# xrgtn/x264-i386pic

Measured on AMD Instinct MI355X. Metric: SAD+SATD candidate-MVs/sec + DCT+quant blocks/sec, 1080p, 1/2/4/8 GPU, higher is better.
Workload: dtype u8; 1 GPU; configs[1]: 1920x1080 luma, full-search ME range 16, sad_16x16 candidate tables, 128 frame pairs per GPU per step; mbs_per_frame=8160, candidates_per_mb=1089, parallelism=frame-per-GPU x1, world_size=1

## Files before the change

x264-i386pic_amd/csrc/me.hip:

```cpp
#include "hipcommon.h"
#include <mutex>
#include <string.h>
#include <stdlib.h>
#include <atomic>
#include <utility>

namespace x264hip {

template <int BD, int R, int P, int Y>
__device__ __forceinline__ void me_row( const typename PT<BD>::pixel *rb, intptr_t rs,
                                        const uint32_t (&F)[16][16 / PT<BD>::PPD], uint32_t (&acc)[16],
                                        typename PT<BD>::sadt *out )
{
    constexpr int NDW = 16 / PT<BD>::PPD;
    constexpr int C0 = Y - 15 > 0 ? Y - 15 : 0;
    constexpr int C1 = Y < 2 * R ? Y : 2 * R;
    uint32_t rr[NDW];
    load_packed<NDW>( rb + (intptr_t)Y * rs, rr );
#pragma unroll
    for( int c = C0; c <= C1; c++ )
    {
        const int r = Y - c;
        uint32_t a = r == 0 ? 0u : acc[c & 15];
#pragma unroll
// ... 479 lines not shown
__global__ __launch_bounds__( 256 ) void me_full_sad16_v5_kernel( const uint16_t *__restrict__ fenc, intptr_t fs,
                                                                  intptr_t ffs, const uint16_t *__restrict__ ref,
                                                                  intptr_t rs, intptr_t rfs, int mbw, int mbh,
                                                                  int nframes, uint32_t *__restrict__ table,
                                                                  const int16_t *__restrict__ centre,
                                                                  int16_t *__restrict__ origin, int xcd )
{
    const me_lane l = me_lane_of<2 * G, true>( xcd, nframes, mbh, mbw );
    if( !l.live )
        return;

    uint32_t F[8][8];
    load_fenc( F, (const uint32_t *)(fenc + l.f * ffs + (intptr_t)(16 * l.mby + 8 * l.h) * fs + 16 * l.mbx),
               (int)(fs / 2) );
    int ox, oy;
    me_window<10, R, P>( centre, l.mb, l.mbx, l.mby, mbw, mbh, ox, oy );
    if( origin && l.grp == 0 && l.h == 0 )
    {
        origin[2 * l.mb] = (int16_t)ox;
        origin[2 * l.mb + 1] = (int16_t)oy;
    }
    const uint32_t *rbase = (const uint32_t *)(ref + l.f * rfs + (intptr_t)(16 * l.mby + 8 * l.h + oy) * rs +
                                               16 * l.mbx + ox + 2 * l.grp);
    uint32_t *out = table + l.mb * ((2 * R + 1) * P) + 2 * l.grp;
    if constexpr( P > 2 * G )
    {
        const int c = 2 * l.grp + l.h;
        if( c <= 2 * R )
            *(uint2 *)(table + l.mb * ((2 * R + 1) * P) + c * P + 2 * G) = make_uint2( 0u, 0u );
    }
    auto store = [out]( int c, uint32_t a0, uint32_t a1 ) { *(uint2 *)(out + c * P) = make_uint2( a0, a1 ); };
    ring_p<ME_LEAD> ring;
    fold_pair fold( F, store );
    me_walk<R, 8, ME_LEAD>( rbase, (int)(rs / 2), ring, fold );
}

template <int R>
__global__ __launch_bounds__( 256 ) void me_full_sad8q_v5_kernel( const uint16_t *__restrict__ fenc, intptr_t fs,
                                                                  intptr_t ffs, const uint16_t *__restrict__ ref,
                                                                  intptr_t rs, intptr_t rfs, int mbw, int mbh,
                                                                  int nframes, uint16_t *__restrict__ table8, int xcd )
{
    constexpr int G = R + 1, P = full_pitch( R );
    const me_lane l = me_lane_of<2 * G, true>( xcd, nframes, mbh, mbw );
    if( !l.live )
        return;
    uint32_t F[8][8];
    load_fenc( F, (const uint32_t *)(fenc + l.f * ffs + (intptr_t)(16 * l.mby + 8 * l.h) * fs + 16 * l.mbx),
               (int)(fs / 2) );
    const uint32_t *rbase = (const uint32_t *)(ref + l.f * rfs + (intptr_t)(16 * l.mby + 8 * l.h - R) * rs +
                                               16 * l.mbx - R + 2 * l.grp);
    uint32_t *ql = (uint32_t *)(table8 + (l.mb * 4 + 2 * l.h) * ((2 * R + 1) * P) + 2 * l.grp);
    uint32_t *qr = ql + (2 * R + 1) * P / 2;
    static_assert( P == 2 * G + 2, "one padding dword per row" );
    for( int c = l.grp; c <= 2 * R; c += G )
    {
        ql[c * (P / 2) + G - l.grp] = 0u;
        qr[c * (P / 2) + G - l.grp] = 0u;
    }
    auto store = [ql, qr]( int c, uint32_t left, uint32_t right ) {
        ql[c * (P / 2)] = left;
        qr[c * (P / 2)] = right;
    };
    ring_p<ME_LEAD> ring;
    fold_quad fold( F, store );
    me_walk<R, 8, ME_LEAD>( rbase, (int)(rs / 2), ring, fold );
}

template <int BD>
hipError_t launch_me_full8( const typename PT<BD>::pixel *fenc, intptr_t fs, intptr_t ffs,
                            const typename PT<BD>::pixel *ref, intptr_t rs, intptr_t rfs, int mbw, int mbh,
                            int nframes, int range, uint16_t *table8, hipStream_t stream )
{
    constexpr int PSZ = sizeof( typename PT<BD>::pixel );
    const int64_t lanes = (int64_t)nframes * mbh * mbw * (BD == 8 ? full_pitch( range ) / 4 : 2 * (range + 1));
    if( lanes <= 0 )
        return hipSuccess;
    if( lanes >= (1ll << 32) || (((uintptr_t)fenc | (uintptr_t)ref | (uintptr_t)(fs * PSZ) | (uintptr_t)(rs * PSZ) |
                                  (uintptr_t)table8) & 3) )
        return hipErrorInvalidValue;
    dim3 blk( 256 ), g( (unsigned)((lanes + 255) / 256) );
    const int xcd = me_xcd();
    switch( range )
    {
#define ME8_CASE( R )                                                                                           \
        case R:                                                                                                 \
            if constexpr( BD == 8 )                                                                             \
                hipLaunchKernelGGL( ( me_full_sad8q_kernel<R> ), g, blk, 0, stream, fenc, fs, ffs, ref, rs, rfs, \
                                    mbw, mbh, nframes, table8, xcd );                                           \
            else                                                                                                \
                hipLaunchKernelGGL( ( me_full_sad8q_v5_kernel<R> ), g, blk, 0, stream, fenc, fs, ffs, ref, rs,  \
                                    rfs, mbw, mbh, nframes, table8, xcd );                                      \
            break;
        ME8_CASE( 4 ) ME8_CASE( 8 ) ME8_CASE( 16 ) ME8_CASE( 24 )
#undef ME8_CASE
        default: return hipErrorInvalidValue;
    }
    return hipGetLastError();
}
X264HIP_INSTANTIATE( launch_me_full8 );

template <int BD>
hipError_t launch_me_full( const typename PT<BD>::pixel *fenc, intptr_t fs, intptr_t ffs,
                           const typename PT<BD>::pixel *ref, intptr_t rs, intptr_t rfs, int mbw, int mbh,
                           int nframes, int range, typename PT<BD>::sadt *table, const int16_t *centre,
                           int16_t *origin, hipStream_t stream )
{
    constexpr int PSZ = sizeof( typename PT<BD>::pixel );
    const bool cen = centre != nullptr;
    const int64_t nmb = (int64_t)nframes * mbh * mbw;
    if( nmb <= 0 )
        return hipSuccess;
    const int ncol = cen ? cen_pitch( BD, range ) : 2 * range + 1;
    const int64_t groups = BD == 8 ? al4( ncol ) / 4 : 2 * (cen ? cen_cols( 10, range ) / 2 : range + 1);
    bool grouped = !(((uintptr_t)fenc | (uintptr_t)ref | (uintptr_t)(fs * PSZ) | (uintptr_t)(rs * PSZ)) & 3);
    if( nmb * groups >= (1ll << 32) )
        grouped = false;
    const bool share = grouped && BD == 8 && !cen && (range == 8 || range == 16);
    const int64_t lanes = nmb * (share ? groups - 1 : grouped ? groups : ncol);
    dim3 blk( 256 ), g( (unsigned)((lanes + 255) / 256) );
    const int xcd = me_xcd();
    switch( range )
    {
#define ME_GO( R, CEN )                                                                                           \
    if( !grouped )                                                                                                \
        hipLaunchKernelGGL( ( me_full_sad16_kernel<BD, R, CEN ? cen_pitch( BD, R ) : 2 * R + 1> ), g, blk, 0,    \
                            stream, fenc, fs, ffs, ref, rs, rfs, mbw, mbh, nframes, table, centre, origin );      \
    else if constexpr( BD == 8 && !CEN && cs_range<R>() )                                                         \
        hipLaunchKernelGGL( ( me_full_sad16_v7_kernel<R, full_pitch( R ) / 4, cs_lanes<R>()> ), g, blk, 0,        \
                            stream, fenc, fs, ffs, ref, rs, rfs, mbw, mbh, nframes, table, centre, origin, xcd ); \
    else if constexpr( BD == 8 )                                                                                  \
        hipLaunchKernelGGL( ( me_full_sad16_v7_kernel<R, (CEN ? cen_pitch( 8, R ) : full_pitch( R )) / 4> ), g,   \
                            blk, 0, stream, fenc, fs, ffs, ref, rs, rfs, mbw, mbh, nframes, table, centre, origin, \
                            xcd );                                                                                \
    else                                                                                                          \
        hipLaunchKernelGGL( ( me_full_sad16_v5_kernel<R, CEN ? cen_cols( 10, R ) / 2 : R + 1,                     \
                                                      CEN ? cen_pitch( 10, R ) : full_pitch( R )> ),              \
                            g, blk, 0, stream, fenc, fs, ffs, ref, rs, rfs, mbw, mbh, nframes, table, centre,     \
                            origin, xcd );
#define ME_CASE( R )                                                                                              \
        case R:                                                                                                   \
            if( cen ) { ME_GO( R, true ) } else { ME_GO( R, false ) }                                             \
            break;
        ME_CASE( 4 ) ME_CASE( 8 ) ME_CASE( 16 ) ME_CASE( 24 )
#undef ME_CASE
#undef ME_GO
        default: return hipErrorInvalidValue;
    }
    return hipGetLastError();
}

X264HIP_INSTANTIATE( launch_me_full );

template <int R> constexpr int esa7_groups() { return ((((2 * R + 3) & ~3) + 3) + 3) / 4; }
template <int R> constexpr int esa7_mbs() { return 256 / esa7_groups<R>(); }
constexpr int esa7_groups_rt( int R ) { return ((((2 * R + 3) & ~3) + 3) + 3) / 4; }
template <int R, bool TAB>
__global__ __launch_bounds__( 256 ) void me_full_esa_v7_kernel( const uint8_t *__restrict__ fenc, intptr_t fs,
                                                                intptr_t ffs, const uint8_t *__restrict__ ref,
                                                                intptr_t rs, intptr_t rfs, int mbw, int mbh,
                                                                int nframes, int me_range,
                                                                const int16_t *__restrict__ par,
                                                                const uint16_t *__restrict__ cost_mv,
                                                                uint32_t *__restrict__ keys, int xcd,
                                                                uint16_t *__restrict__ tab,
                                                                int16_t *__restrict__ torg,
                                                                const int32_t *__restrict__ init_cost )
{
    constexpr int G = esa7_groups<R>();
    constexpr int P = cen_pitch( 8, R );
    constexpr int W = 2 * R + 1;
    constexpr int MPW = esa7_mbs<R>();
    constexpr int NSP = 256 - MPW * G;
    constexpr int SP = W | 1;
    __shared__ uint32_t s_row[MPW * SP];
    __shared__ uint32_t s_need[MPW];
    __shared__ uint32_t s_key[MPW];
    const uint32_t nmb = (uint32_t)nframes * (uint32_t)mbh * (uint32_t)mbw;
    const int tid = (int)threadIdx.x;
    const bool spare = tid >= MPW * G;
    const uint32_t wg0 = (xcd ? xcd_block( blockIdx.x, gridDim.x ) : blockIdx.x) * MPW;

    int lmb, grp, mbx, mby, bmx, bmy, min_x, min_y, max_x, max_y, width, ox, oy;
    int64_t mb, f;
    bool live;
    const uint16_t *cx, *cy;
    auto setup = [&]( int slot ) __attribute__( ( always_inline ) ) {
        lmb = slot;
        const uint32_t mbr = wg0 + (uint32_t)slot;
        live = mbr < nmb;
        const uint32_t mb32 = min( mbr, nmb - 1 ), t32 = mb32 / (uint32_t)mbw, f32 = t32 / (uint32_t)mbh;
        mbx = (int)(mb32 - t32 * (uint32_t)mbw);
        mby = (int)(t32 - f32 * (uint32_t)mbh);
        mb = mb32;
        f = f32;
        const int16_t *p = par + 8 * mb;
        bmx = p[0];
        bmy = p[1];
        min_x = max( bmx - me_range, (int)p[4] );
        min_y = max( bmy - me_range, (int)p[5] );
        max_x = min( bmx + me_range, (int)p[6] );
        max_y = min( bmy + me_range, (int)p[7] );
        width = (max_x - min_x + 3) & ~3;
        cx = cost_mv - p[2];
        cy = cost_mv - p[3];
        const int16_t cen[2] = { (int16_t)bmx, (int16_t)bmy };
        me_window<8, R, P>( cen, 0, mbx, mby, mbw, mbh, ox, oy );
    };
    setup( spare ? 0 : tid / G );
    grp = spare ? G : tid - lmb * G;
    const bool need = live && min_x + width - 1 - ox >= 4 * G;
    if( !spare && grp == 0 )
    {
        s_need[lmb] = need;
        s_key[lmb] = 0xFFFFFFFFu;
    }
    if( TAB && !spare && live && grp == 0 )
    {
        torg[2 * mb] = (int16_t)ox;
        torg[2 * mb + 1] = (int16_t)oy;
    }
    if( !TAB && !spare && live )
    {
        uint32_t *srow = s_row + lmb * SP;
#pragma unroll
        for( int c0 = 0; c0 < W; c0 += G )
        {
            const int c = c0 + grp, my = oy + c;
            if( c < W )
                srow[c] = my >= min_y && my <= max_y
                              ? ((uint32_t)cy[4 * my] << 12) + (uint32_t)((my - min_y) * width)
                              : 0xFFFFFFFFu;
        }
    }
    __syncthreads();
    bool twice = false;
    if constexpr( NSP > 0 )
    {
        if( spare )
        {
            int k = tid - MPW * G, slot = -1;
            for( int i = 0; i < MPW && slot < 0; i++ )
                if( s_need[i] && k-- == 0 )
                    slot = i;
            if( slot >= 0 )
                setup( slot );
            else
                live = false;
        }
        else if( grp == 0 && need )
        {
            int rank = 0;
            for( int i = 0; i < lmb; i++ )
                rank += s_need[i] ? 1 : 0;
            twice = rank >= NSP;
        }
    }
    else
        twice = !spare && grp == 0 && need;

    uint32_t F[16][4];
    load_fenc( F, (const uint32_t *)(fenc + f * ffs + (intptr_t)(16 * mby) * fs + 16 * mbx), (int)(fs / 4) );
    const uint32_t *rmb = (const uint32_t *)(ref + f * rfs + (intptr_t)(16 * mby + oy) * rs + 16 * mbx + ox);
    uint32_t ck[4];
    auto columns = [&]( int g ) __attribute__( ( always_inline ) ) {
#pragma unroll
        for( int k = 0; k < 4; k++ )
        {
            const int mx = ox + 4 * g + k;
            const bool in = mx >= min_x && mx < min_x + width;
            ck[k] = in ? ((uint32_t)cx[mx * 4] << 12) + (uint32_t)(mx - min_x) : 0xF0000000u;
        }
    };
    columns( grp );
    uint32_t key = 0xFFFFFFFFu;
    uint32_t *srow = s_row + lmb * SP;
    auto reduce = [&]( int c, uint32_t lo, uint32_t hi ) {
        __attribute__( ( address_space( 3 ) ) ) uint32_t *q = (__attribute__( ( address_space( 3 ) ) ) uint32_t *)srow;
        asm volatile( "" : "+v"( q ) );
        const uint32_t S = q[c];
        uint32_t w0 = lo & 0xffff, w1 = lo >> 16, w2 = hi & 0xffff, w3 = hi >> 16;
        asm( "" : "+v"( w0 ), "+v"( w1 ), "+v"( w2 ), "+v"( w3 ) );
        const uint32_t k0 = __builtin_elementwise_add_sat( (w0 << 12) + ck[0], S );
        const uint32_t k1 = __builtin_elementwise_add_sat( (w1 << 12) + ck[1], S );
        const uint32_t k2 = __builtin_elementwise_add_sat( (w2 << 12) + ck[2], S );
        const uint32_t k3 = __builtin_elementwise_add_sat( (w3 << 12) + ck[3], S );
        key = min( min( key, k0 ), k1 );
        key = min( min( key, k2 ), k3 );
        asm volatile( "" : "+v"( key ) );
    };
    ring_q<ME_LEAD> ring;
    if constexpr( TAB )
    {
        uint64_t *out = (uint64_t *)(tab + mb * ((2 * R + 1) * P) + 4 * grp);
        auto store = [&out]( int c, uint32_t lo, uint32_t hi ) { out[c * (P / 4)] = ((uint64_t)hi << 32) | lo; };
        fold_row fold( F, store );
        if( live )
        {
            me_walk<R, 16, ME_LEAD>( rmb + grp, (int)(rs / 4), ring, fold );
            if( twice )
            {
                out = (uint64_t *)(tab + mb * ((2 * R + 1) * P) + 4 * G);
                me_walk<R, 16, ME_LEAD>( rmb + G, (int)(rs / 4), ring, fold );
            }
        }
    }
    else
    {
        fold_row fold( F, reduce );
        me_walk<R, 16, ME_LEAD>( rmb + grp, (int)(rs / 4), ring, fold );
        if( twice )
        {
            columns( G );
            me_walk<R, 16, ME_LEAD>( rmb + G, (int)(rs / 4), ring, fold );
        }
        if( live && key < 0xF0000000u )
            atomicMin( &s_key[lmb], key );
        __syncthreads();
        if( tid < MPW && wg0 + (uint32_t)tid < nmb )
        {
            const int64_t i = wg0 + (uint32_t)tid;
            const int16_t *q = par + 8 * i;
            const int qx = q[0], qy = q[1];
            const int mnx = max( qx - me_range, (int)q[4] ), mny = max( qy - me_range, (int)q[5] );
            const int wd = (min( qx + me_range, (int)q[6] ) - mnx + 3) & ~3;
            const uint32_t k = s_key[tid];
            int32_t bc = init_cost[i], rx = qx, ry = qy;
            if( k != 0xFFFFFFFFu && (int32_t)(k >> 12) < bc )
            {
                const int ki = (int)(k & 4095);
                bc = (int32_t)(k >> 12);
                ry = mny + ki / wd;
                rx = mnx + ki % wd;
            }
            keys[3 * i] = (uint32_t)bc;
            keys[3 * i + 1] = (uint32_t)rx;
            keys[3 * i + 2] = (uint32_t)ry;
        }
    }
}

__global__ __launch_bounds__( 256 ) void me_esa_finish_kernel( int nmb, int me_range, const int16_t *__restrict__ par,
                                                               const int32_t *__restrict__ init_cost,
                                                               int32_t *__restrict__ out )
{
    const int i = blockIdx.x * blockDim.x + threadIdx.x;
    if( i >= nmb )
        return;
    const int16_t *p = par + 8 * i;
    const int bmx = p[0], bmy = p[1];
    const int min_x = max( bmx - me_range, (int)p[4] ), min_y = max( bmy - me_range, (int)p[5] );
    const int max_x = min( bmx + me_range, (int)p[6] );
    const int width = (max_x - min_x + 3) & ~3;
    const uint32_t key = (uint32_t)out[3 * i];
    int32_t bcost = init_cost[i], rx = bmx, ry = bmy;
    if( key != 0xFFFFFFFFu && (int32_t)(key >> 12) < bcost )
    {
        const int k = (int)(key & 4095);
        bcost = (int32_t)(key >> 12);
        ry = min_y + k / width;
        rx = min_x + k % width;
    }
    out[3 * i] = bcost;
    out[3 * i + 1] = rx;
    out[3 * i + 2] = ry;
}

template <int R>
__global__ __launch_bounds__( 256 ) void me_full_esa_v5_kernel( const uint16_t *__restrict__ fenc, intptr_t fs,
                                                                intptr_t ffs, const uint16_t *__restrict__ ref,
                                                                intptr_t rs, intptr_t rfs, int mbw, int mbh,
                                                                int nframes, int me_range,
                                                                const int16_t *__restrict__ par,
                                                                const uint16_t *__restrict__ cost_mv,
                                                                uint32_t *__restrict__ keys, int xcd )
{
    constexpr int G = cen_cols( 10, R ) / 2;
    constexpr int P = cen_pitch( 10, R );
    const int64_t slot = (int64_t)(xcd ? xcd_block( blockIdx.x, gridDim.x ) : blockIdx.x) * blockDim.x + threadIdx.x;
    const int64_t total = (int64_t)nframes * mbh * mbw * (2 * G);
    if( slot >= total )
        return;
    const int h = (int)(slot & 1);
    const int grp = (int)((slot >> 1) % G);
    const int64_t mb = slot / (2 * G);
    const int mbx = (int)(mb % mbw);
    const int64_t t = mb / mbw;
    const int mby = (int)(t % mbh);
    const int64_t f = t / mbh;

    uint32_t F[8][8];
    load_fenc( F, (const uint32_t *)(fenc + f * ffs + (intptr_t)(16 * mby + 8 * h) * fs + 16 * mbx), (int)(fs / 2) );
    const int16_t *p = par + 8 * mb;
    const int bmx = p[0], bmy = p[1];
    const int min_x = max( bmx - me_range, (int)p[4] ), min_y = max( bmy - me_range, (int)p[5] );
    const int max_x = min( bmx + me_range, (int)p[6] ), max_y = min( bmy + me_range, (int)p[7] );
    const int width = (max_x - min_x + 3) & ~3;
    const uint16_t *cx = cost_mv - p[2], *cy = cost_mv - p[3];
    int ox, oy;
    const int16_t cen[2] = { (int16_t)bmx, (int16_t)bmy };
    me_window<10, R, P>( cen, 0, mbx, mby, mbw, mbh, ox, oy );
    const uint32_t *rbase =
        (const uint32_t *)(ref + f * rfs + (intptr_t)(16 * mby + 8 * h + oy) * rs + 16 * mbx + ox + 2 * grp);
    const int mxc = ox + 2 * grp + h;
    const bool cin = mxc >= min_x && mxc < min_x + width;
    const uint32_t cinv = cin ? 0u : 0xFFFFFFFFu;
    const int ccost = cin ? (int)cx[mxc * 4] : 0;
    uint32_t key = 0xFFFFFFFFu;
    const int ibase = mxc - min_x - min_y * width;
    uint32_t ynext = cy[4 * min( max( oy, min_y ), max_y )];
    auto reduce = [&]( int c, uint32_t a0, uint32_t a1 ) {
        const int my = oy + c;
        const uint32_t rinv = my >= min_y && my <= max_y ? 0u : 0xFFFFFFFFu;
        const uint32_t ycost = ynext;
        int yi = 4 * min( max( my + 1, min_y ), max_y );
        asm volatile( "" : "+v"( yi ) );
        ynext = cy[yi];
        const uint32_t sad = h ? a1 : a0;
        const uint32_t k = ((sad + (uint32_t)ccost + ycost) << 12) | (uint32_t)(my * width + ibase);
        key = min( key, k | cinv | rinv );
        asm volatile( "" : "+v"( key ) );
    };
    ring_p<ME_LEAD> ring;
    fold_pair fold( F, reduce );
    me_walk<R, 8, ME_LEAD>( rbase, (int)(rs / 2), ring, fold );
    key = min( key, (uint32_t)__builtin_amdgcn_update_dpp( (int)0xFFFFFFFF, (int)key, 0xB1, 0xF, 0xF, false ) );
    if( !h && key != 0xFFFFFFFFu )
        atomicMin( keys + 3 * mb, key );
}

template <int BD>
hipError_t launch_me_search_esa( const typename PT<BD>::pixel *fenc, intptr_t fs, intptr_t ffs,
                                 const typename PT<BD>::pixel *ref, intptr_t rs, intptr_t rfs, int mbw, int mbh,
                                 int nframes, int range, int me_range, const int16_t *par, const int32_t *init_cost,
                                 const uint16_t *cost_mv, int32_t *out, hipStream_t stream )
{
    const int64_t nmb = (int64_t)nframes * mbw * mbh;
    if( nmb <= 0 )
        return hipSuccess;
    if( nmb > 0x7fffffff ||
        (((uintptr_t)fenc | (uintptr_t)ref | (uintptr_t)(fs * sizeof( typename PT<BD>::pixel )) |
          (uintptr_t)(rs * sizeof( typename PT<BD>::pixel ))) & 3) )
        return hipErrorInvalidValue;
    if( BD != 8 )
    {
        const hipError_t e = hipMemsetAsync( out, 0xFF, (size_t)nmb * 3 * sizeof( int32_t ), stream );
        if( e != hipSuccess )
            return e;
    }
    const int64_t mpw = range == 4 ? esa7_mbs<4>() : range == 8 ? esa7_mbs<8>() : range == 16 ? esa7_mbs<16>()
                                                                                               : esa7_mbs<24>();
    const int64_t lanes = nmb * 2 * (cen_cols( 10, range ) / 2);
    dim3 blk( 256 ), g( (unsigned)(BD == 8 ? (nmb + mpw - 1) / mpw : (lanes + 255) / 256) );
    const int xcd = me_xcd();
    switch( range )
    {
#define ESA_CASE( R )                                                                                             \
        case R:                                                                                                   \
            if constexpr( BD == 8 )                                                                               \
                hipLaunchKernelGGL( ( me_full_esa_v7_kernel<R, false> ), g, blk, 0, stream, fenc, fs, ffs, ref, rs, \
                                    rfs, mbw, mbh, nframes, me_range, par, cost_mv, (uint32_t *)out, xcd,         \
                                    nullptr, nullptr, init_cost );                                                \
            else                                                                                                  \
                hipLaunchKernelGGL( ( me_full_esa_v5_kernel<R> ), g, blk, 0, stream, fenc, fs, ffs, ref, rs, rfs, \
                                    mbw, mbh, nframes, me_range, par, cost_mv, (uint32_t *)out, xcd );            \
            break;
        ESA_CASE( 4 ) ESA_CASE( 8 ) ESA_CASE( 16 ) ESA_CASE( 24 )
#undef ESA_CASE
// ... 584 lines not shown
            nmvsad--;
            if( lane == 0 )
                mvsads[bi] = mvsads[nmvsad];
        }
        tesa_wave_sync();
    }

    uint32_t best = 0xFFFFFFFFu;
    for( int u0 = 0; any( u0 < nmvsad * 8 ); u0 += SEG )
    {
        const int u = u0 + lane, k = u >> 3, part = u & 7;
        uint32_t v = 0;
        int cmx = 0, cmy = 0;
        if( k < nmvsad )
        {
            const E e = mvsads[k];
            cmx = emx( e );
            cmy = emy( e );
            const int bx = 8 * (part & 1), by = 4 * (part >> 1);
            constexpr int HDW = 8 / PT<BD>::PPD;
            uint32_t a[4][HDW], rr[4][HDW];
            const pixel *rp = p_fref + (intptr_t)(cmy + by) * rs + cmx + bx;
#pragma unroll
            for( int y = 0; y < 4; y++ )
            {
                load_row_u<HDW>( rp + y * rs, rr[y] );
#pragma unroll
                for( int j = 0; j < HDW; j++ )
                    a[y][j] = fl[(by + y) * NDW + bx / PT<BD>::PPD + j];
            }
            if( satd )
                v = satd8x4_packed<BD>( a, rr ) >> 1;
            else
            {
#pragma unroll
                for( int y = 0; y < 4; y++ )
#pragma unroll
                    for( int j = 0; j < HDW; j++ )
                        v = sadp<BD>( a[y][j], rr[y][j], v );
            }
        }
        v += (uint32_t)__builtin_amdgcn_update_dpp( 0, (int)v, 0xB1, 0xF, 0xF, false );
        v += (uint32_t)__builtin_amdgcn_update_dpp( 0, (int)v, 0x4E, 0xF, 0xF, false );
        v += (uint32_t)__builtin_amdgcn_update_dpp( 0, (int)v, 0x12C, 0xF, 0xF, false );
        if( k < nmvsad && part == 0 )
        {
            const uint32_t cost = v + cx[cmx * 4] + cy[cmy * 4];
            best = min( best, (cost << 6) | (uint32_t)k );
        }
    }
    best = seg_lane<SEG>( seg_scan_min<SEG>( best ), SEG - 1, sg );
    if( lane == 0 && live && mbo < nmb )
    {
        int32_t bcost = init_cost[mb], rx = bmx0, ry = bmy0;
        if( best != 0xFFFFFFFFu && (int32_t)(best >> 6) < bcost )
        {
            const E e = mvsads[best & 63];
            bcost = (int32_t)(best >> 6);
            rx = emx( e );
            ry = emy( e );
        }
        out[4 * mb] = bcost;
        out[4 * mb + 1] = rx;
        out[4 * mb + 2] = ry;
        out[4 * mb + 3] = nmvsad;
    }
}

template <int BD, int NR, int SEG, bool TAB, bool SPEC = false>
__global__ __launch_bounds__( 64 ) __attribute__( ( amdgpu_waves_per_eu( TESA_WPE ) ) ) void me_tesa_kernel( const typename PT<BD>::pixel *__restrict__ fenc, intptr_t fs,
                                                        intptr_t ffs, const typename PT<BD>::pixel *__restrict__ ref,
                                                        intptr_t rs, intptr_t rfs,
                                                        const uint16_t *__restrict__ integral, intptr_t ifs, int mbw,
                                                        int mbh, int nmb, int me_range, int satd,
                                                        const typename PT<BD>::sadt *__restrict__ table, int R,
                                                        int tcols, int tpitch, const int16_t *__restrict__ origin,
                                                        const int16_t *__restrict__ par,
                                                        const int32_t *__restrict__ init_cost,
                                                        const uint16_t *__restrict__ cost_mv, int32_t *__restrict__ out,
                                                        int cap )
{
    constexpr int NDW = 16 / PT<BD>::PPD;
    constexpr int NSEG = 64 / SEG;
    extern __shared__ uint64_t tesa_lds[];
    __shared__ uint32_t fls[NSEG][16 * NDW];
    const int sg = (int)threadIdx.x / SEG, lane = (int)threadIdx.x % SEG;
    const int64_t mbo = (int64_t)blockIdx.x * NSEG + sg;
    const int64_t mb = mbo < nmb ? mbo : nmb - 1;
    const int ox = origin ? origin[2 * mb] : -R, oy = origin ? origin[2 * mb + 1] : -R;
    tesa_scan_mb<BD, NR, SEG, TAB, SPEC>( fenc, fs, ffs, ref, rs, rfs, integral, ifs, mbw, mbh, nmb, me_range, satd,
                                          table, R, tcols, tpitch, ox, oy, par, init_cost, cost_mv, out, mbo, true, sg,
                                          lane, (tesa_ent<SEG> *)tesa_lds + (int64_t)sg * cap, fls[sg] );
}

__global__ __launch_bounds__( 256 ) void tesa_centre_kernel( int nmb, const int16_t *__restrict__ par,
                                                             int16_t *__restrict__ centre )
{
    const int i = blockIdx.x * blockDim.x + threadIdx.x;
    if( i < nmb )
    {
        centre[2 * i] = par[8 * i];
        centre[2 * i + 1] = par[8 * i + 1];
    }
}

static std::mutex g_pool_mu;
static hipMemPool_t g_pools[64] = {};
hipError_t scratch_alloc( void **p, size_t bytes, hipStream_t stream )
{
    int dev = 0;
    hipError_t e = stream_device( stream, &dev );
    if( e != hipSuccess )
        return e;
    if( dev < 0 || dev >= 64 )
        return hipErrorInvalidDevice;
    hipMemPool_t pool;
    {
        std::lock_guard<std::mutex> lk( g_pool_mu );
        if( !g_pools[dev] )
        {
            hipMemPoolProps props;
            memset( &props, 0, sizeof( props ) );
            props.allocType = hipMemAllocationTypePinned;
            props.handleTypes = hipMemHandleTypeNone;
            props.location.type = hipMemLocationTypeDevice;
            props.location.id = dev;
            if( (e = hipMemPoolCreate( &g_pools[dev], &props )) != hipSuccess )
            {
                g_pools[dev] = nullptr;
                return e;
            }
            uint64_t thr = UINT64_MAX;
            (void)hipMemPoolSetAttribute( g_pools[dev], hipMemPoolAttrReleaseThreshold, &thr );
        }
        pool = g_pools[dev];
    }
    return hipMallocFromPoolAsync( p, bytes, pool, stream );
}

hipError_t scratch_trim( int dev )
{
    std::lock_guard<std::mutex> lk( g_pool_mu );
    for( int d = 0; d < 64; d++ )
        if( g_pools[d] && (dev < 0 || dev == d) )
        {
            const hipError_t e = hipMemPoolTrimTo( g_pools[d], 0 );
            if( e != hipSuccess )
                return e;
        }
    return hipSuccess;
}

template <int BD>
hipError_t launch_me_tesa( const typename PT<BD>::pixel *fenc, intptr_t fs, intptr_t ffs,
                           const typename PT<BD>::pixel *ref, intptr_t rs, intptr_t rfs, const uint16_t *integral,
                           intptr_t ifs, int mbw, int mbh, int nframes, int me_range, int satd,
                           const typename PT<BD>::sadt *table, int R, const int16_t *origin, const int16_t *par,
                           const int32_t *init_cost, const uint16_t *cost_mv, int32_t *out, hipStream_t stream )
{
    const int64_t nmb = (int64_t)nframes * mbw * mbh;
    if( nmb <= 0 )
        return hipSuccess;
    if( me_range < 1 || me_range > 32 || nmb > 0x7fffffff || rs <= 0 || rs >= (1 << 18) )
        return hipErrorInvalidValue;
    if( !table && me_range <= 24 && variant( V_TESA ) != 1 )
    {
        using sadt = typename PT<BD>::sadt;
        const int TR = me_range <= 4 ? 4 : me_range <= 8 ? 8 : me_range <= 16 ? 16 : 24;
        const size_t tab = (size_t)nmb * (2 * TR + 1) * (size_t)cen_pitch( BD, TR ) * sizeof( sadt );
        const size_t bytes = tab + (size_t)nmb * 8;
        void *buf = nullptr;
        if( scratch_alloc( &buf, bytes, stream ) == hipSuccess )
        {
            sadt *ttab = (sadt *)buf;
            int16_t *cen = (int16_t *)((uint8_t *)buf + tab), *org = cen + 2 * nmb;
            hipLaunchKernelGGL( tesa_centre_kernel, dim3( (unsigned)((nmb + 255) / 256) ), dim3( 256 ), 0, stream,
                                (int)nmb, par, cen );
            hipError_t e = hipGetLastError();
            if( e == hipSuccess )
            {
                if constexpr( BD == 8 )
                {
                    switch( TR )
                    {
#define TT_CASE( RR )                                                                                             \
                        case RR:                                                                                  \
                            hipLaunchKernelGGL( ( me_full_esa_v7_kernel<RR, true> ),                              \
                                                dim3( (unsigned)((nmb + esa7_mbs<RR>() - 1) / esa7_mbs<RR>()) ),  \
                                                dim3( 256 ), 0, stream, fenc, fs, ffs, ref, rs, rfs, mbw, mbh,    \
                                                nframes, me_range, par, cost_mv, nullptr, me_xcd(), ttab, org,    \
                                                nullptr );                                                        \
                            break;
                        TT_CASE( 4 ) TT_CASE( 8 ) TT_CASE( 16 ) TT_CASE( 24 )
#undef TT_CASE
                    }
                    e = hipGetLastError();
                }
                else
                    e = launch_me_full<BD>( fenc, fs, ffs, ref, rs, rfs, mbw, mbh, nframes, TR, ttab, cen, org, stream );
            }
            if( e == hipSuccess )
                e = launch_me_tesa<BD>( fenc, fs, ffs, ref, rs, rfs, integral, ifs, mbw, mbh, nframes, me_range, satd,
                                        ttab, TR, org, par, init_cost, cost_mv, out, stream );
            const hipError_t f = hipFreeAsync( buf, stream );
            return e != hipSuccess ? e : f;
        }
        (void)hipGetLastError();
    }

    const int cap = (2 * me_range + 1) * ((2 * me_range + 3) & ~3);
    const int tcols = origin ? cen_cols( BD, R ) : 2 * R + 1;
    const int tpitch = origin ? cen_pitch( BD, R ) : full_pitch( R );
    if( table && (R < 1 || tpitch > 64) )
        return hipErrorInvalidValue;
#define TESA_GO( NR, SEG, T )                                                                                    \
    hipLaunchKernelGGL( ( me_tesa_kernel<BD, NR, SEG, T, T> ), dim3( (unsigned)((nmb + 64 / SEG - 1) / (64 / SEG)) ), \
                        dim3( 64 ), (64 / SEG) * (size_t)cap * (SEG == 32 ? 4 : 8), stream, fenc, fs, ffs, ref, rs, \
                        rfs, integral, ifs, mbw, mbh, (int)nmb, me_range, satd, table, R, tcols, tpitch, origin, par, \
                        init_cost, cost_mv, out, cap )
    if( me_range <= 16 )
    {
        if( table ) { TESA_GO( 33, 32, true ); } else { TESA_GO( 33, 32, false ); }
    }
    else
    {
        if( table ) { TESA_GO( 65, 64, true ); } else { TESA_GO( 65, 64, false ); }
    }
#undef TESA_GO
    return hipGetLastError();
}

X264HIP_INSTANTIATE( launch_me_tesa );

__host__ __device__ constexpr int esa8_part( int h, int s ) { return s == 0 ? 4 + 2 * h : s == 1 ? 5 + 2 * h : s == 2 ? h : 2 + h; }
template <int R> constexpr int esa8_groups() { return R / 2; }
template <int BD, int R> constexpr int esa8_lgroups() { return BD == 8 ? esa8_groups<R>() : R + 1; }
template <int BD, int R> constexpr int esa8_mbs() { return 256 / (2 * esa8_lgroups<BD, R>()); }

__device__ __forceinline__ uint32_t esa8_mad( uint32_t v, uint32_t c, uint32_t s4096, bool hi )
{
    uint32_t d;
    if( hi )
        asm( "v_mad_u32_u16 %0, %1, %2, %3 op_sel:[1,0,0,0]" : "=v"( d ) : "v"( v ), "s"( s4096 ), "v"( c ) );
    else
        asm( "v_mad_u32_u16 %0, %1, %2, %3" : "=v"( d ) : "v"( v ), "s"( s4096 ), "v"( c ) );
    return d;
}

typedef uint16_t u16x2 __attribute__( ( ext_vector_type( 2 ) ) );
__device__ __forceinline__ uint64_t pk_add_u16x4( uint64_t a, uint64_t b )
{
    const u16x2 lo = __builtin_bit_cast( u16x2, (uint32_t)a ) + __builtin_bit_cast( u16x2, (uint32_t)b );
    const u16x2 hi = __builtin_bit_cast( u16x2, (uint32_t)(a >> 32) ) + __builtin_bit_cast( u16x2, (uint32_t)(b >> 32) );
    return ((uint64_t)__builtin_bit_cast( uint32_t, hi ) << 32) | __builtin_bit_cast( uint32_t, lo );
}

template <int BD, int NDW, int PH, int CH>
__device__ __forceinline__ uint32_t esa8_scan( const typename PT<BD>::pixel *fb, intptr_t fs,
                                               const typename PT<BD>::pixel *rb, intptr_t rs, const uint16_t *cx,
                                               const uint16_t *cy, int lane, int nt, int nb, int nl, int nr, int wd,
                                               int lw, int rw, int x0, int y0, int iy0, int iy1, int ix1, int min_x,
                                               int min_y, int width, uint32_t key )
{
    uint32_t a[PH][NDW];
#pragma unroll
    for( int y = 0; y < PH; y++ )
#pragma unroll
        for( int k = 0; k < NDW; k++ )
            a[y][k] = ((const uint32_t *)(fb + y * fs))[k];
    const int nc = nt + nb + nl + nr;
    for( int u = lane; u < nc; u += 64 )
    {
        int mx, my, v = u;
        if( v < nt )
            my = y0 + v / wd, mx = x0 + v % wd;
        else if( (v -= nt) < nb )
            my = iy1 + 1 + v / wd, mx = x0 + v % wd;
        else if( (v -= nb) < nl )
            my = iy0 + v / lw, mx = x0 + v % lw;
        else
            v -= nl, my = iy0 + v / rw, mx = ix1 + 1 + v % rw;
        const typename PT<BD>::pixel *r = rb + (intptr_t)my * rs + mx;
        uint32_t sad = 0;
#pragma unroll
        for( int y0r = 0; y0r < PH; y0r += CH )
        {
            uint32_t b[CH][NDW];
#pragma unroll
            for( int y = 0; y < CH; y++ )
                load_packed<NDW>( r + (y0r + y) * rs, b[y] );
#pragma unroll
            for( int y = 0; y < CH; y++ )
#pragma unroll
                for( int k = 0; k < NDW; k++ )
                    sad = sadp<BD>( a[y0r + y][k], b[y][k], sad );
        }
        const uint32_t idx = (uint32_t)((my - min_y) * width + mx - min_x);
        key = min( key, ((sad + cx[4 * mx] + cy[4 * my]) << 12) | idx );
    }
    return key;
}

template <int NDW, int PH>
__device__ __forceinline__ uint32_t esa8_scan4( const uint8_t *fb, intptr_t fs, const uint8_t *rb, intptr_t rs,
                                                const uint16_t *cx, const uint16_t *cy, int lane, int y0, int y1,
                                                int iy0, int iy1, int ix0, int ix1, int x0, int width, int min_x,
                                                int min_y, uint32_t key )
{
    uint32_t a[PH][NDW];
#pragma unroll
    for( int y = 0; y < PH; y++ )
#pragma unroll
        for( int k = 0; k < NDW; k++ )
            a[y][k] = ((const uint32_t *)(fb + y * fs))[k];
    if( width <= 0 || y1 < y0 )
        return key;
    const int x1 = x0 + width - 1, ng = width >> 2;
    const int gl = (ix0 - x0 + 3) >> 2, gr0 = (ix1 + 1 - x0) >> 2, gr = ix1 + 1 <= x1 ? ng - gr0 : 0;
    const int mh = iy1 - iy0 + 1;
    const int nt = (iy0 - y0) * ng, nb = (y1 - iy1) * ng, nl = mh * gl, nr = mh * gr;
    const int nu = nt + nb + nl + nr;
    for( int u = lane; u < nu; u += 64 )
    {
        int my, g, v = u;
        if( v < nt )
            my = y0 + v / ng, g = v % ng;
        else if( (v -= nt) < nb )
            my = iy1 + 1 + v / ng, g = v % ng;
        else if( (v -= nb) < nl )
            my = iy0 + v / gl, g = v % gl;
        else
            v -= nl, my = iy0 + v / gr, g = gr0 + v % gr;
        const int gx = x0 + 4 * g;
        const uint8_t *r = rb + (intptr_t)my * rs + gx;
        const uint32_t sh = (uint32_t)((uintptr_t)r & 3);
        uint64_t acc = 0;
#pragma unroll
        for( int y = 0; y < PH; y++ )
        {
            const uint32_t *base = (const uint32_t *)(r + y * rs - sh);
            uint32_t w[NDW + 2], d[NDW + 1];
#pragma unroll
            for( int k = 0; k <= NDW; k++ )
                w[k] = base[k];
            w[NDW + 1] = base[sh ? NDW + 1 : NDW];
#pragma unroll
            for( int k = 0; k <= NDW; k++ )
                d[k] = __builtin_amdgcn_alignbyte( w[k + 1], w[k], sh );
#pragma unroll
            for( int k = 0; k < NDW; k++ )
                acc = __builtin_amdgcn_qsad_pk_u16_u8( (uint64_t)d[k + 1] << 32 | d[k], a[y][k], acc );
        }
        const uint32_t rowc = cy[4 * my], rowi = (uint32_t)((my - min_y) * width + gx - min_x);
#pragma unroll
        for( int k = 0; k < 4; k++ )
        {
            const uint32_t sad = (uint32_t)(acc >> (16 * k)) & 0xffff;
            key = min( key, ((sad + cx[4 * (gx + k)] + rowc) << 12) | (rowi + k) );
        }
    }
    return key;
}

template <int BD, int CH>
__device__ __forceinline__ void esa8_direct( const typename PT<BD>::pixel *__restrict__ fenc, intptr_t fs,
                                             intptr_t ffs, const typename PT<BD>::pixel *__restrict__ ref,
                                             intptr_t rs, intptr_t rfs, int mbw, int mbh, int me_range,
                                             const int16_t *__restrict__ par, const int32_t *__restrict__ init_cost,
                                             const uint16_t *__restrict__ cost_mv, int32_t *__restrict__ out,
                                             int64_t i, uint32_t key, int tx0, int tx1, int ty0, int ty1, int lane )
{
    using pixel = typename PT<BD>::pixel;
    constexpr int PPD = PT<BD>::PPD;
    const int64_t mb = i >> 3;
    const int p = (int)(i & 7);
    const int64_t t = mb / mbw;
    const int mbx = (int)(mb - t * mbw), mby = (int)(t % mbh);
    const int64_t f = t / mbh;
    const int16_t *q = par + 8 * i;
    const int bmx = q[0], bmy = q[1];
    const int min_x = max( bmx - me_range, (int)q[4] ), min_y = max( bmy - me_range, (int)q[5] );
    const int max_x = min( bmx + me_range, (int)q[6] ), max_y = min( bmy + me_range, (int)q[7] );
// ... 321 lines not shown
```

Before: 507.1 billion SAD16x16 candidates/s.

## Simplify ESA v7 to fixed 2R-column window with unaligned ring loads

Shrinks the ESA v7 search table to exactly 2R columns per MB row. It centres the window on the clamped search range and loads reference rows with a sub-dword shift ring, so groups no longer need 4-byte alignment padding. This removes the spare-thread redistribution, the second walk for overflow columns, a shared-memory need array and, in table mode, a barrier. The table-mode path also drops the separate centre kernel launch for 8-bit. The risks are edge columns not being covered when the range is not aligned, and the extra cost of unaligned shifts.

```diff
diff --git a/x264-i386pic_amd/csrc/me.hip b/x264-i386pic_amd/csrc/me.hip
--- a/x264-i386pic_amd/csrc/me.hip
+++ b/x264-i386pic_amd/csrc/me.hip
@@ -655,9 +655,8 @@
 
 X264HIP_INSTANTIATE( launch_me_full );
 
-template <int R> constexpr int esa7_groups() { return ((((2 * R + 3) & ~3) + 3) + 3) / 4; }
+template <int R> constexpr int esa7_groups() { return 2 * R / 4; }
 template <int R> constexpr int esa7_mbs() { return 256 / esa7_groups<R>(); }
-constexpr int esa7_groups_rt( int R ) { return ((((2 * R + 3) & ~3) + 3) + 3) / 4; }
 template <int R, bool TAB>
 __global__ __launch_bounds__( 256 ) void me_full_esa_v7_kernel( const uint8_t *__restrict__ fenc, intptr_t fs,
                                                                 intptr_t ffs, const uint8_t *__restrict__ ref,
@@ -671,59 +670,38 @@
                                                                 const int32_t *__restrict__ init_cost )
 {
     constexpr int G = esa7_groups<R>();
-    constexpr int P = cen_pitch( 8, R );
+    constexpr int P = 2 * R;
     constexpr int W = 2 * R + 1;
     constexpr int MPW = esa7_mbs<R>();
-    constexpr int NSP = 256 - MPW * G;
     constexpr int SP = W | 1;
     __shared__ uint32_t s_row[MPW * SP];
-    __shared__ uint32_t s_need[MPW];
     __shared__ uint32_t s_key[MPW];
     const uint32_t nmb = (uint32_t)nframes * (uint32_t)mbh * (uint32_t)mbw;
     const int tid = (int)threadIdx.x;
-    const bool spare = tid >= MPW * G;
+    const bool idle = tid >= MPW * G;
     const uint32_t wg0 = (xcd ? xcd_block( blockIdx.x, gridDim.x ) : blockIdx.x) * MPW;
-
-    int lmb, grp, mbx, mby, bmx, bmy, min_x, min_y, max_x, max_y, width, ox, oy;
-    int64_t mb, f;
-    bool live;
-    const uint16_t *cx, *cy;
-    auto setup = [&]( int slot ) __attribute__( ( always_inline ) ) {
-        lmb = slot;
-        const uint32_t mbr = wg0 + (uint32_t)slot;
-        live = mbr < nmb;
-        const uint32_t mb32 = min( mbr, nmb - 1 ), t32 = mb32 / (uint32_t)mbw, f32 = t32 / (uint32_t)mbh;
-        mbx = (int)(mb32 - t32 * (uint32_t)mbw);
-        mby = (int)(t32 - f32 * (uint32_t)mbh);
-        mb = mb32;
-        f = f32;
-        const int16_t *p = par + 8 * mb;
-        bmx = p[0];
-        bmy = p[1];
-        min_x = max( bmx - me_range, (int)p[4] );
-        min_y = max( bmy - me_range, (int)p[5] );
-        max_x = min( bmx + me_range, (int)p[6] );
-        max_y = min( bmy + me_range, (int)p[7] );
-        width = (max_x - min_x + 3) & ~3;
-        cx = cost_mv - p[2];
-        cy = cost_mv - p[3];
-        const int16_t cen[2] = { (int16_t)bmx, (int16_t)bmy };
-        me_window<8, R, P>( cen, 0, mbx, mby, mbw, mbh, ox, oy );
-    };
-    setup( spare ? 0 : tid / G );
-    grp = spare ? G : tid - lmb * G;
-    const bool need = live && min_x + width - 1 - ox >= 4 * G;
-    if( !spare && grp == 0 )
-    {
-        s_need[lmb] = need;
+    const int lmb = idle ? 0 : tid / G, grp = idle ? 0 : tid - lmb * G;
+    const uint32_t mbr = wg0 + (uint32_t)lmb;
+    const bool live = !idle && mbr < nmb;
+    const uint32_t mb32 = min( mbr, nmb - 1 ), t32 = mb32 / (uint32_t)mbw, f32 = t32 / (uint32_t)mbh;
+    const int mbx = (int)(mb32 - t32 * (uint32_t)mbw), mby = (int)(t32 - f32 * (uint32_t)mbh);
+    const int64_t mb = mb32, f = f32;
+    const int16_t *p = par + 8 * mb;
+    const int bmx = p[0], bmy = p[1];
+    const int min_x = max( bmx - me_range, (int)p[4] ), min_y = max( bmy - me_range, (int)p[5] );
+    const int max_x = min( bmx + me_range, (int)p[6] ), max_y = min( bmy + me_range, (int)p[7] );
+    const int width = (max_x - min_x + 3) & ~3;
+    const uint16_t *cx = cost_mv - p[2], *cy = cost_mv - p[3];
+    int ox, oy;
+    me_window( R, P, 0, min_x + R, bmy, mbx, mby, mbw, mbh, ox, oy );
+    if( !TAB && !idle && grp == 0 )
         s_key[lmb] = 0xFFFFFFFFu;
-    }
-    if( TAB && !spare && live && grp == 0 )
+    if( TAB && live && grp == 0 )
     {
         torg[2 * mb] = (int16_t)ox;
         torg[2 * mb + 1] = (int16_t)oy;
     }
-    if( !TAB && !spare && live )
+    if( !TAB && live )
     {
         uint32_t *srow = s_row + lmb * SP;
 #pragma unroll
@@ -736,87 +714,51 @@
                               : 0xFFFFFFFFu;
         }
     }
-    __syncthreads();
-    bool twice = false;
-    if constexpr( NSP > 0 )
-    {
-        if( spare )
-        {
-            int k = tid - MPW * G, slot = -1;
-            for( int i = 0; i < MPW && slot < 0; i++ )
-                if( s_need[i] && k-- == 0 )
-                    slot = i;
-            if( slot >= 0 )
-                setup( slot );
-            else
-                live = false;
-        }
-        else if( grp == 0 && need )
-        {
-            int rank = 0;
-            for( int i = 0; i < lmb; i++ )
-                rank += s_need[i] ? 1 : 0;
-            twice = rank >= NSP;
-        }
-    }
-    else
-        twice = !spare && grp == 0 && need;
+    if constexpr( !TAB )
+        __syncthreads();
 
     uint32_t F[16][4];
     load_fenc( F, (const uint32_t *)(fenc + f * ffs + (intptr_t)(16 * mby) * fs + 16 * mbx), (int)(fs / 4) );
-    const uint32_t *rmb = (const uint32_t *)(ref + f * rfs + (intptr_t)(16 * mby + oy) * rs + 16 * mbx + ox);
-    uint32_t ck[4];
-    auto columns = [&]( int g ) __attribute__( ( always_inline ) ) {
-#pragma unroll
-        for( int k = 0; k < 4; k++ )
-        {
-            const int mx = ox + 4 * g + k;
-            const bool in = mx >= min_x && mx < min_x + width;
-            ck[k] = in ? ((uint32_t)cx[mx * 4] << 12) + (uint32_t)(mx - min_x) : 0xF0000000u;
-        }
-    };
-    columns( grp );
-    uint32_t key = 0xFFFFFFFFu;
-    uint32_t *srow = s_row + lmb * SP;
-    auto reduce = [&]( int c, uint32_t lo, uint32_t hi ) {
-        __attribute__( ( address_space( 3 ) ) ) uint32_t *q = (__attribute__( ( address_space( 3 ) ) ) uint32_t *)srow;
-        asm volatile( "" : "+v"( q ) );
-        const uint32_t S = q[c];
-        uint32_t w0 = lo & 0xffff, w1 = lo >> 16, w2 = hi & 0xffff, w3 = hi >> 16;
-        asm( "" : "+v"( w0 ), "+v"( w1 ), "+v"( w2 ), "+v"( w3 ) );
-        const uint32_t k0 = __builtin_elementwise_add_sat( (w0 << 12) + ck[0], S );
-        const uint32_t k1 = __builtin_elementwise_add_sat( (w1 << 12) + ck[1], S );
-        const uint32_t k2 = __builtin_elementwise_add_sat( (w2 << 12) + ck[2], S );
-        const uint32_t k3 = __builtin_elementwise_add_sat( (w3 << 12) + ck[3], S );
-        key = min( min( key, k0 ), k1 );
-        key = min( min( key, k2 ), k3 );
-        asm volatile( "" : "+v"( key ) );
-    };
-    ring_q<ME_LEAD> ring;
+    const uint32_t *rbase =
+        (const uint32_t *)(ref + f * rfs + (intptr_t)(16 * mby + oy) * rs + 16 * mbx + (ox & ~3)) + grp;
+    ring_qu<ME_LEAD> ring;
+    ring.sh = (uint32_t)ox & 3;
     if constexpr( TAB )
     {
-        uint64_t *out = (uint64_t *)(tab + mb * ((2 * R + 1) * P) + 4 * grp);
+        uint64_t *out = (uint64_t *)(tab + mb * (W * P) + 4 * grp);
         auto store = [&out]( int c, uint32_t lo, uint32_t hi ) { out[c * (P / 4)] = ((uint64_t)hi << 32) | lo; };
         fold_row fold( F, store );
         if( live )
-        {
-            me_walk<R, 16, ME_LEAD>( rmb + grp, (int)(rs / 4), ring, fold );
-            if( twice )
-            {
-                out = (uint64_t *)(tab + mb * ((2 * R + 1) * P) + 4 * G);
-                me_walk<R, 16, ME_LEAD>( rmb + G, (int)(rs / 4), ring, fold );
-            }
-        }
+            me_walk<R, 16, ME_LEAD>( rbase, (int)(rs / 4), ring, fold );
     }
     else
     {
+        uint32_t ck[4];
+#pragma unroll
+        for( int k = 0; k < 4; k++ )
+        {
+            const int mx = ox + 4 * grp + k;
+            const bool in = mx >= min_x && mx < min_x + width;
+            ck[k] = in ? ((uint32_t)cx[mx * 4] << 12) + (uint32_t)(mx - min_x) : 0xF0000000u;
+        }
+        uint32_t key = 0xFFFFFFFFu;
+        uint32_t *srow = s_row + lmb * SP;
+        auto reduce = [&]( int c, uint32_t lo, uint32_t hi ) {
+            __attribute__( ( address_space( 3 ) ) ) uint32_t *q = (__attribute__( ( address_space( 3 ) ) ) uint32_t *)srow;
+            asm volatile( "" : "+v"( q ) );
+            const uint32_t S = q[c];
+            uint32_t w0 = lo & 0xffff, w1 = lo >> 16, w2 = hi & 0xffff, w3 = hi >> 16;
+            asm( "" : "+v"( w0 ), "+v"( w1 ), "+v"( w2 ), "+v"( w3 ) );
+            const uint32_t k0 = __builtin_elementwise_add_sat( (w0 << 12) + ck[0], S );
+            const uint32_t k1 = __builtin_elementwise_add_sat( (w1 << 12) + ck[1], S );
+            const uint32_t k2 = __builtin_elementwise_add_sat( (w2 << 12) + ck[2], S );
+            const uint32_t k3 = __builtin_elementwise_add_sat( (w3 << 12) + ck[3], S );
+            key = min( min( key, k0 ), k1 );
+            key = min( min( key, k2 ), k3 );
+            asm volatile( "" : "+v"( key ) );
+        };
         fold_row fold( F, reduce );
-        me_walk<R, 16, ME_LEAD>( rmb + grp, (int)(rs / 4), ring, fold );
-        if( twice )
-        {
-            columns( G );
-            me_walk<R, 16, ME_LEAD>( rmb + G, (int)(rs / 4), ring, fold );
-        }
+        me_walk<R, 16, ME_LEAD>( rbase, (int)(rs / 4), ring, fold );
         if( live && key < 0xF0000000u )
             atomicMin( &s_key[lmb], key );
         __syncthreads();
@@ -1707,65 +1649,14 @@
 }
 
 template <int BD>
-hipError_t launch_me_tesa( const typename PT<BD>::pixel *fenc, intptr_t fs, intptr_t ffs,
-                           const typename PT<BD>::pixel *ref, intptr_t rs, intptr_t rfs, const uint16_t *integral,
-                           intptr_t ifs, int mbw, int mbh, int nframes, int me_range, int satd,
-                           const typename PT<BD>::sadt *table, int R, const int16_t *origin, const int16_t *par,
-                           const int32_t *init_cost, const uint16_t *cost_mv, int32_t *out, hipStream_t stream )
-{
-    const int64_t nmb = (int64_t)nframes * mbw * mbh;
-    if( nmb <= 0 )
-        return hipSuccess;
-    if( me_range < 1 || me_range > 32 || nmb > 0x7fffffff || rs <= 0 || rs >= (1 << 18) )
-        return hipErrorInvalidValue;
-    if( !table && me_range <= 24 && variant( V_TESA ) != 1 )
-    {
-        using sadt = typename PT<BD>::sadt;
-        const int TR = me_range <= 4 ? 4 : me_range <= 8 ? 8 : me_range <= 16 ? 16 : 24;
-        const size_t tab = (size_t)nmb * (2 * TR + 1) * (size_t)cen_pitch( BD, TR ) * sizeof( sadt );
-        const size_t bytes = tab + (size_t)nmb * 8;
-        void *buf = nullptr;
-        if( scratch_alloc( &buf, bytes, stream ) == hipSuccess )
-        {
-            sadt *ttab = (sadt *)buf;
-            int16_t *cen = (int16_t *)((uint8_t *)buf + tab), *org = cen + 2 * nmb;
-            hipLaunchKernelGGL( tesa_centre_kernel, dim3( (unsigned)((nmb + 255) / 256) ), dim3( 256 ), 0, stream,
-                                (int)nmb, par, cen );
-            hipError_t e = hipGetLastError();
-            if( e == hipSuccess )
-            {
-                if constexpr( BD == 8 )
-                {
-                    switch( TR )
-                    {
-#define TT_CASE( RR )                                                                                             \
-                        case RR:                                                                                  \
-                            hipLaunchKernelGGL( ( me_full_esa_v7_kernel<RR, true> ),                              \
-                                                dim3( (unsigned)((nmb + esa7_mbs<RR>() - 1) / esa7_mbs<RR>()) ),  \
-                                                dim3( 256 ), 0, stream, fenc, fs, ffs, ref, rs, rfs, mbw, mbh,    \
-                                                nframes, me_range, par, cost_mv, nullptr, me_xcd(), ttab, org,    \
-                                                nullptr );                                                        \
-                            break;
-                        TT_CASE( 4 ) TT_CASE( 8 ) TT_CASE( 16 ) TT_CASE( 24 )
-#undef TT_CASE
-                    }
-                    e = hipGetLastError();
-                }
-                else
-                    e = launch_me_full<BD>( fenc, fs, ffs, ref, rs, rfs, mbw, mbh, nframes, TR, ttab, cen, org, stream );
-            }
-            if( e == hipSuccess )
-                e = launch_me_tesa<BD>( fenc, fs, ffs, ref, rs, rfs, integral, ifs, mbw, mbh, nframes, me_range, satd,
-                                        ttab, TR, org, par, init_cost, cost_mv, out, stream );
-            const hipError_t f = hipFreeAsync( buf, stream );
-            return e != hipSuccess ? e : f;
-        }
-        (void)hipGetLastError();
-    }
-
+static hipError_t launch_tesa_scan( const typename PT<BD>::pixel *fenc, intptr_t fs, intptr_t ffs,
+                                    const typename PT<BD>::pixel *ref, intptr_t rs, intptr_t rfs,
+                                    const uint16_t *integral, intptr_t ifs, int mbw, int mbh, int64_t nmb, int me_range,
+                                    int satd, const typename PT<BD>::sadt *table, int R, int tcols, int tpitch,
+                                    const int16_t *origin, const int16_t *par, const int32_t *init_cost,
+                                    const uint16_t *cost_mv, int32_t *out, hipStream_t stream )
+{
     const int cap = (2 * me_range + 1) * ((2 * me_range + 3) & ~3);
-    const int tcols = origin ? cen_cols( BD, R ) : 2 * R + 1;
-    const int tpitch = origin ? cen_pitch( BD, R ) : full_pitch( R );
     if( table && (R < 1 || tpitch > 64) )
         return hipErrorInvalidValue;
 #define TESA_GO( NR, SEG, T )                                                                                    \
@@ -1783,6 +1674,71 @@
     }
 #undef TESA_GO
     return hipGetLastError();
+}
+
+template <int BD>
+hipError_t launch_me_tesa( const typename PT<BD>::pixel *fenc, intptr_t fs, intptr_t ffs,
+                           const typename PT<BD>::pixel *ref, intptr_t rs, intptr_t rfs, const uint16_t *integral,
+                           intptr_t ifs, int mbw, int mbh, int nframes, int me_range, int satd,
+                           const typename PT<BD>::sadt *table, int R, const int16_t *origin, const int16_t *par,
+                           const int32_t *init_cost, const uint16_t *cost_mv, int32_t *out, hipStream_t stream )
+{
+    const int64_t nmb = (int64_t)nframes * mbw * mbh;
+    if( nmb <= 0 )
+        return hipSuccess;
+    if( me_range < 1 || me_range > 32 || nmb > 0x7fffffff || rs <= 0 || rs >= (1 << 18) )
+        return hipErrorInvalidValue;
+    if( !table && me_range <= 24 && variant( V_TESA ) != 1 )
+    {
+        using sadt = typename PT<BD>::sadt;
+        const int TR = me_range <= 4 ? 4 : me_range <= 8 ? 8 : me_range <= 16 ? 16 : 24;
+        const int tcols = BD == 8 ? 2 * TR : cen_cols( BD, TR ), tpitch = BD == 8 ? 2 * TR : cen_pitch( BD, TR );
+        const size_t tab = (size_t)nmb * (2 * TR + 1) * (size_t)tpitch * sizeof( sadt );
+        const size_t bytes = tab + (size_t)nmb * 8;
+        void *buf = nullptr;
+        if( scratch_alloc( &buf, bytes, stream ) == hipSuccess )
+        {
+            sadt *ttab = (sadt *)buf;
+            int16_t *cen = (int16_t *)((uint8_t *)buf + tab), *org = cen + 2 * nmb;
+            hipError_t e = hipSuccess;
+            if constexpr( BD == 8 )
+            {
+                switch( TR )
+                {
+#define TT_CASE( RR )                                                                                             \
+                    case RR:                                                                                      \
+                        hipLaunchKernelGGL( ( me_full_esa_v7_kernel<RR, true> ),                                  \
+                                            dim3( (unsigned)((nmb + esa7_mbs<RR>() - 1) / esa7_mbs<RR>()) ),      \
+                                            dim3( 256 ), 0, stream, fenc, fs, ffs, ref, rs, rfs, mbw, mbh,        \
+                                            nframes, me_range, par, cost_mv, nullptr, me_xcd(), ttab, org,        \
+                                            nullptr );                                                            \
+                        break;
+                    TT_CASE( 4 ) TT_CASE( 8 ) TT_CASE( 16 ) TT_CASE( 24 )
+#undef TT_CASE
+                }
+                e = hipGetLastError();
+            }
+            else
+            {
+                hipLaunchKernelGGL( tesa_centre_kernel, dim3( (unsigned)((nmb + 255) / 256) ), dim3( 256 ), 0, stream,
+                                    (int)nmb, par, cen );
+                e = hipGetLastError();
+                if( e == hipSuccess )
+                    e = launch_me_full<BD>( fenc, fs, ffs, ref, rs, rfs, mbw, mbh, nframes, TR, ttab, cen, org, stream );
+            }
+            if( e == hipSuccess )
+                e = launch_tesa_scan<BD>( fenc, fs, ffs, ref, rs, rfs, integral, ifs, mbw, mbh, nmb, me_range, satd,
+                                          ttab, TR, tcols, tpitch, org, par, init_cost, cost_mv, out, stream );
+            const hipError_t f = hipFreeAsync( buf, stream );
+            return e != hipSuccess ? e : f;
+        }
+        (void)hipGetLastError();
+    }
+
+    const int tcols = origin ? cen_cols( BD, R ) : 2 * R + 1;
+    const int tpitch = origin ? cen_pitch( BD, R ) : full_pitch( R );
+    return launch_tesa_scan<BD>( fenc, fs, ffs, ref, rs, rfs, integral, ifs, mbw, mbh, nmb, me_range, satd, table, R,
+                                 tcols, tpitch, origin, par, init_cost, cost_mv, out, stream );
 }
 
 X264HIP_INSTANTIATE( launch_me_tesa );
```

Result: no change. 505.7 billion SAD16x16 candidates/s (-0.3%).
